# weigert/SoilMachine

Hardware: NVIDIA H100
Metric: particle-steps/sec (higher is better)
Workload: dtype f64

## Files before the change

soilmachine_b200/csrc/sm_device.cuh:

```cuda
#pragma once
#include <cuda_runtime.h>
#include "sm_core.cuh"

#ifdef SM_PROFILE
#define SM_PROF_DECL unsigned long long prof_[16] = {0}; long long pt_ = clock64();
#define SM_PROF(i) { long long t_ = clock64(); prof_[i] += (unsigned long long)(t_ - pt_); pt_ = t_; }
#define SM_PROF_FLUSH(ctl) { for (int i_ = 0; i_ < 16; i_++) if (prof_[i_]) atomicAdd(&(ctl)->prof[i_], prof_[i_]); }
#else
#define SM_PROF_DECL
#define SM_PROF(i)
#define SM_PROF_FLUSH(ctl)
#endif

struct PoolRing {
  unsigned long long head;
  unsigned long long tail;
};

struct RunCtl {
  unsigned int barrier;
  unsigned int alive_slot[3];
  unsigned int tag_base;
  unsigned int err;
  unsigned long long steps, sweeps, exit_oob, exit_evap, exit_stall, drops, alive;
// ... 96 lines not shown
__device__ __forceinline__ unsigned int ld_relaxed_sys_u32(const unsigned int* p) {
  unsigned int v;
  asm volatile("ld.relaxed.sys.global.u32 %0, [%1];" : "=r"(v) : "l"(p) : "memory");
  return v;
}
__device__ __forceinline__ unsigned long long ld_relaxed_sys_u64(const unsigned long long* p) {
  unsigned long long v;
  asm volatile("ld.relaxed.sys.global.u64 %0, [%1];" : "=l"(v) : "l"(p) : "memory");
  return v;
}
__device__ __forceinline__ void prefetch_l2(const void* p) { asm volatile("prefetch.global.L2 [%0];" ::"l"(p)); }
#ifndef SM_POLL_NS
#define SM_POLL_NS 0
#endif
__device__ __forceinline__ void poll_backoff() { if (SM_POLL_NS > 0) __nanosleep(SM_POLL_NS); }
__device__ __forceinline__ unsigned int ld_acquire_sys_u32(const unsigned int* p) {
  unsigned int v;
  asm volatile("ld.acquire.sys.global.u32 %0, [%1];" : "=r"(v) : "l"(p) : "memory");
  return v;
}
__device__ __forceinline__ void st_release_sys_u32(unsigned int* p, unsigned int v) {
  asm volatile("st.release.sys.global.u32 [%0], %1;" ::"l"(p), "r"(v) : "memory");
}

__device__ __forceinline__ unsigned long long ld_acquire_sys_u64(const unsigned long long* p) {
  unsigned long long v;
  asm volatile("ld.acquire.sys.global.u64 %0, [%1];" : "=l"(v) : "l"(p) : "memory");
  return v;
}
__device__ __forceinline__ void st_release_sys_u64(unsigned long long* p, unsigned long long v) {
  asm volatile("st.release.sys.global.u64 [%0], %1;" ::"l"(p), "l"(v) : "memory");
}

__device__ __forceinline__ void grid_barrier(unsigned int* counter, unsigned int& epoch) {
  __syncthreads();
  epoch++;
  if (threadIdx.x == 0) {
    __threadfence();
    atomicAdd(counter, 1u);
    const unsigned int target = epoch * gridDim.x;
    while ((int)(ld_relaxed_u32(counter) - target) < 0) poll_backoff();
    __threadfence();
  }
  __syncthreads();
}

__device__ __forceinline__ unsigned int grid_barrier_multi(const DevCtx& c, unsigned int& epoch, unsigned int gbase,
                                                           unsigned int local_alive_slot) {
  RunCtl* ctl = c.ctl;
  __syncthreads();
  epoch++;
  const unsigned int ge = gbase + epoch;
  if (threadIdx.x == 0) {
    __threadfence();
    atomicAdd(&ctl->barrier, 1u);
    if (blockIdx.x == 0) {
      const unsigned int target = epoch * gridDim.x;
      while ((int)(ld_acquire_u32(&ctl->barrier) - target) < 0) { }
      const unsigned int mine = ld_volatile_u32(&ctl->alive_slot[local_alive_slot]);
#ifdef SM_XBAR_FENCES
      for (int q = 0; q < c.nranks; q++) st_volatile_u32(&c.peer[q].ctl->xalive[ge & 1u][c.rank], mine);
      __threadfence_system();
      for (int q = 0; q < c.nranks; q++) st_volatile_u32(&c.peer[q].ctl->xflag[c.rank], ge);
      unsigned int total = 0;
      for (int q = 0; q < c.nranks; q++) {
        while ((int)(ld_volatile_u32(&ctl->xflag[q]) - ge) < 0) { }
      }
      __threadfence_system();
      for (int q = 0; q < c.nranks; q++) total += ld_volatile_u32(&ctl->xalive[ge & 1u][q]);
#else
      for (int q = 0; q < c.nranks; q++) st_volatile_u32(&c.peer[q].ctl->xalive[ge & 1u][c.rank], mine);
      for (int q = 0; q < c.nranks; q++) st_release_sys_u32(&c.peer[q].ctl->xflag[c.rank], ge);
      unsigned int total = 0;
      for (int q = 0; q < c.nranks; q++) {
        while ((int)(ld_acquire_sys_u32(&ctl->xflag[q]) - ge) < 0) { }
// ... 260 lines not shown
```

soilmachine_b200/csrc/sm_engine.cu:

```cuda
#include <cuda_runtime.h>
#include <stddef.h>
#include <stdio.h>
#include <stdlib.h>
#include <string.h>
#include <string>
#include <vector>
#include <algorithm>
#include "../../include/soilmachine_b200.h"
#include "../../include/soilmachine/soilfile.hpp"
#include "sm_device.cuh"
#include "sm_noise.cuh"
#include "sm_hydro.cuh"
#include "sm_lbm.cuh"

#define KIND_WATER 0
#define KIND_WIND 1

template <int KIND> struct Reach {
  static constexpr int D = (KIND == KIND_WATER) ? 6 : 10;
  static constexpr int G = (KIND == KIND_WATER) ? 8 : 16;
  static constexpr int STEP = (KIND == KIND_WATER) ? 2 : 3;
  static constexpr int RING = (KIND == KIND_WATER) ? 1 : 2;
};

// ... 1756 lines not shown
    if (mask & (1 << kind)) {
      for (int ls = lshift;; ls--) {
        const size_t sm2 = (size_t)(threads >> ls) * (SM_WIN_BYTES + SM_KX * 4);
        int occ = 0;
        if (kind == KIND_WATER) CK(cudaOccupancyMaxActiveBlocksPerMultiprocessor(&occ, k_run_exact<KIND_WATER>, threads, sm2));
        else CK(cudaOccupancyMaxActiveBlocksPerMultiprocessor(&occ, k_run_exact<KIND_WIND>, threads, sm2));
        const long long need_threads = (long long)std::max(n, 1) << ls;
        const long long maxblocks = (long long)ctx->num_sms * occ;
        if (occ >= 1 && (need_threads <= maxblocks * threads || ls == 0)) {
          use_exact = true; lshift = ls; smem = sm2;
          blocks = (int)std::max<long long>(1, std::min<long long>(maxblocks, (need_threads + threads - 1) / threads));
          break;
        }
        if (ls == 0) break;
      }
    }
  }
  bool use_coop = SM_DEFAULT_COOP || ctx->d.bud != nullptr || ctx->d.wind_v4 != nullptr;
  {
    const char* e = getenv("SM_KERNEL");
    if (e && strcmp(e, "thread") == 0) use_coop = false;
    if (e && strcmp(e, "warp") == 0) use_coop = true;
  }
  if (use_coop) {
    const int sw_warps = kind == KIND_WIND ? SwShape<KIND_WIND>::WARPS : SwShape<KIND_WATER>::WARPS;
    const int cthreads = sw_warps * 32;
    int occ = 0;
    const bool budget = ctx->d.bud != nullptr;
    bool exact = false;
    {
      const char* e = getenv("SM_EXACT");
      exact = (((e ? atoi(e) : SM_DEFAULT_EXACT) >> kind) & 1) != 0;
    }
    void* const fns[16] = {(void*)k_sweep<KIND_WATER, false, false, false>, (void*)k_sweep<KIND_WIND, false, false, false>,
                           (void*)k_sweep<KIND_WATER, true, false, false>,  (void*)k_sweep<KIND_WIND, true, false, false>,
                           (void*)k_sweep<KIND_WATER, false, true, false>,  (void*)k_sweep<KIND_WIND, false, true, false>,
                           (void*)k_sweep<KIND_WATER, true, true, false>,   (void*)k_sweep<KIND_WIND, true, true, false>,
                           (void*)k_sweep<KIND_WATER, false, false, true>,  (void*)k_sweep<KIND_WIND, false, false, true>,
                           (void*)k_sweep<KIND_WATER, true, false, true>,   (void*)k_sweep<KIND_WIND, true, false, true>,
                           (void*)k_sweep<KIND_WATER, false, true, true>,   (void*)k_sweep<KIND_WIND, false, true, true>,
                           (void*)k_sweep<KIND_WATER, true, true, true>,    (void*)k_sweep<KIND_WIND, true, true, true>};
    void* fn = fns[(exact ? 8 : 0) + (budget ? 4 : 0) + (multi ? 2 : 0) + (kind == KIND_WATER ? 0 : 1)];
    const size_t csmem = (size_t)2 * (((size_t)std::max(n, 1) + 31) / 32) * sizeof(unsigned int);
    if (csmem > 40 * 1024) CK(cudaFuncSetAttribute((const void*)fn, cudaFuncAttributeMaxDynamicSharedMemorySize, (int)csmem));
    CK(cudaOccupancyMaxActiveBlocksPerMultiprocessor(&occ, (const void*)fn, cthreads, csmem));
    if (occ < 1) return fail(ctx, SM_ERR_CUDA, "sweep kernel does not fit an SM");
    const long long maxblocks = std::max<long long>(1, (long long)ctx->num_sms * occ / ctx->share);
    const long long want = ((long long)std::max(n, 1) + sw_warps - 1) / sw_warps;
    const int cblocks = (int)std::max<long long>(1, std::min(maxblocks, want));
    DevCtx dd = ctx->d;
    int ms = max_sweeps;
    if (ms <= 0) ms = -1;
    if (max_sweeps == SM_SWEEPS_NONE) ms = 0;
    void* cargs[] = {&dd, &n, (void*)&d_spawn, &ms};
    CK(cudaMemsetAsync(ctx->d.ctl, 0, 4 * sizeof(unsigned int), ctx->stream));
    CK(cudaMemsetAsync(&ctx->d.ctl->ticket[0], 0, 3 * sizeof(unsigned int), ctx->stream));
    for (int i = 0; i < 3; i++)
      CK(cudaMemsetAsync(ctx->d.lmask[i], 0, ((size_t)ctx->max_particles / 32 + 2) * sizeof(unsigned int), ctx->stream));
    CK(cudaEventRecord(ctx->ev0, ctx->stream));
    CK(cudaLaunchCooperativeKernel(fn, dim3(cblocks), dim3(cthreads), cargs, csmem, ctx->stream));
    CK(cudaEventRecord(ctx->ev1, ctx->stream));
    ctx->launches++;
    ctx->timing_pending = true;
    return SM_OK;
  }
  DevCtx d = ctx->d;
  if (max_sweeps <= 0) max_sweeps = -1;
  if (max_sweeps == SM_SWEEPS_NONE) max_sweeps = 0;
  void* args[] = {&d, &n, (void*)&d_spawn, &max_sweeps, &lshift};
  CK(cudaMemsetAsync(ctx->d.ctl, 0, 4 * sizeof(unsigned int), ctx->stream));
  CK(cudaEventRecord(ctx->ev0, ctx->stream));
  if (multi && kind == KIND_WATER)
    CK(cudaLaunchCooperativeKernel((void*)k_run<KIND_WATER, true>, dim3(blocks), dim3(threads), args, smem, ctx->stream));
  else if (multi)
    CK(cudaLaunchCooperativeKernel((void*)k_run<KIND_WIND, true>, dim3(blocks), dim3(threads), args, smem, ctx->stream));
  else if (use_exact && kind == KIND_WATER)
    CK(cudaLaunchCooperativeKernel((void*)k_run_exact<KIND_WATER>, dim3(blocks), dim3(threads), args, smem, ctx->stream));
  else if (use_exact)
    CK(cudaLaunchCooperativeKernel((void*)k_run_exact<KIND_WIND>, dim3(blocks), dim3(threads), args, smem, ctx->stream));
  else if (kind == KIND_WATER)
    CK(cudaLaunchCooperativeKernel((void*)k_run<KIND_WATER, false>, dim3(blocks), dim3(threads), args, smem, ctx->stream));
// ... 547 lines not shown
```

soilmachine_b200/csrc/sm_sweep.cuh:

```cuda
#pragma once
#include "sm_coop.cuh"

template <int KIND> struct SwShape {
  static constexpr int WARPS = (KIND == KIND_WIND) ? 10 : 8;
  static constexpr int MINBLOCKS = (KIND == KIND_WIND) ? 2 : 3;
};
#define SM_SW_NEAR 31
#define SM_SW_NEARX 128

struct WarpDev {
  int lane;
  template <class F> __device__ __forceinline__ void each(int n, F f) {
    __syncwarp();
    if (lane < n) f(lane);
    __syncwarp();
  }
  template <class F> __device__ __forceinline__ unsigned int ballot(int n, F f) {
    __syncwarp();
    bool v = false;
    if (lane < n) v = f(lane);
    const unsigned int m = __ballot_sync(0xffffffffu, v);
    __syncwarp();
    return m;
  }
  template <class F> __device__ __forceinline__ void one(F f) {
    __syncwarp();
    if (lane == 0) f();
    __syncwarp();
  }
  __device__ __forceinline__ bool lead() const { return lane == 0; }
};

template <bool MULTI, bool BUDGET = false> struct DevBack {
  static constexpr bool kBudget = BUDGET;
  static constexpr bool kHydroHooks = false;
  __device__ __forceinline__ void air_mark(Sec32*, int, int) {}
  __device__ __forceinline__ void wet_mark(int, int) {}
  __device__ __forceinline__ double volume_factor() const { return c.volume_factor; }
  const DevCtx& c;
  const SoilDev* s_soils;
  unsigned int phase;
  int cur_q;
  __device__ __forceinline__ DevBack(const DevCtx& ctx, const SoilDev* ss, unsigned int tag)
      : c(ctx), s_soils(ss), phase(tag % 3u), cur_q(0) {}
  __device__ __forceinline__ int dimx() const { return c.dimx; }
  __device__ __forceinline__ int dimy() const { return c.dimy; }
  __device__ __forceinline__ int scale() const { return c.scale; }
  __device__ __forceinline__ const SoilDev* soilp(uint32_t t) const { return &s_soils[t]; }
  __device__ __forceinline__ Sec32* cell_ptr(int x, int y) const { return ::cell_ptr<MULTI>(c, x, y); }
  __device__ __forceinline__ void focus(int x, int) { if (MULTI) cur_q = owner_of_x<true>(c, x); }
  __device__ __forceinline__ Sec32 pool_load(uint32_t i) { return MULTI ? c.peer[cur_q].pool[i] : c.pool[i]; }
  __device__ __forceinline__ void pool_store(uint32_t i, const Sec32& r) {
    if (MULTI) c.peer[cur_q].pool[i] = r; else c.pool[i] = r;
  }
  __device__ uint32_t pool_alloc() {
    const unsigned int pr = (phase + 1u) % 3u;
    RunCtl* const ctl = MULTI ? c.peer[cur_q].ctl : c.ctl;
    uint32_t* const ring = MULTI ? c.peer[cur_q].ringbuf[pr] : c.ringbuf[pr];
    const unsigned long long cap = MULTI ? c.peer[cur_q].pool_cap : c.pool_cap;
    PoolRing* R = &ctl->ring[pr];
    const unsigned long long t = *((volatile unsigned long long*)&R->tail);
    if (*((volatile unsigned long long*)&R->head) < t) {
      const unsigned long long h = MULTI ? atomicAdd_system(&R->head, 1ull) : atomicAdd(&R->head, 1ull);
      if (h < t) return ring[h % cap];
// ... 15 lines not shown
  }
  __device__ __forceinline__ float wfreq(int i) const { return c.wfreq[i]; }
  __device__ __forceinline__ float wtrack(int i) const { return c.wtrack[i]; }
  __device__ __forceinline__ float windfreq(int i) const { return c.windfreq[i]; }
  __device__ __forceinline__ void set_wtrack(int i, float v) { c.wtrack[i] = v; }
  __device__ __forceinline__ void set_windfreq(int i, float v) { c.windfreq[i] = v; }
  __device__ __forceinline__ void note_transfer() {}
  __device__ __forceinline__ void pspeed(float px, float py, double height, float* ps) const {
    const WindField f{c.wind_v4, c.wind_nx, c.wind_ny, c.wind_nz, c.dimx, c.dimy, c.scale};
    wind_field_pspeed(f, px, py, height, ps);
  }
};

struct __align__(32) WarpSmem {
  CoopScratch cs;
  uint32_t blk[SM_SW_NEARX];
  uint32_t pred[12];
  uint32_t cnt;
  uint32_t m0[SM_SW_NEARX / 32];
  uint32_t n1[SM_SW_NEARX / 32];
  uint32_t remote;
  uint32_t succ;
  uint32_t blkxy[SM_SW_NEARX];
};

#ifndef SM_PREFETCH
#define SM_PREFETCH 1
#endif
__device__ __forceinline__ float next_dy(const WaterP& p) { return p.sy; }
__device__ __forceinline__ float next_dy(const WindP& p) { return p.sz; }
template <class W, class A> __device__ __forceinline__ int do_step_coop(W& w, A& a, WaterP& p) { return water_step_coop(w, a, p); }
template <class W, class A> __device__ __forceinline__ int do_step_coop(W& w, A& a, WindP& p) { return wind_step_coop(w, a, p); }

template <int KIND, bool MULTI, bool EXACT = false>
__device__ __forceinline__ uint32_t coop_scan(const DevCtx& c, WarpSmem& ws, int lane, unsigned int tag, int pid, int ix,
                                              int iy, int R) {
  const unsigned int par = tag & 1u;
  const int G = Reach<KIND>::G;
  const int nbx = (c.dimx + G - 1) / G, nby = (c.dimy + G - 1) / G;
  if (lane == 0) { ws.cnt = 0; ws.succ = 0; if (EXACT) ws.remote = 0; }
  if (EXACT && lane < SM_SW_NEARX / 32) ws.m0[lane] = 0;
  __syncwarp();
  if (lane < 9) {
    const int cx = ix / G + lane / 3 - 1, cy = iy / G + lane % 3 - 1;
    uint32_t best = SM_NIL;
    if (cx >= 0 && cx < nbx && cy >= 0 && cy < nby) {
      const int bq = MULTI ? owner_of_x<MULTI>(c, cx * G) : 0;
      const unsigned long long* hp = MULTI ? c.peer[bq].head[par] : c.head[par];
      const unsigned long long h = *((volatile const unsigned long long*)&hp[cx * nby + cy]);
      if ((unsigned int)(h >> 32) == tag) {
        const uint2* nodes = MULTI ? c.peer[bq].node[par] : c.node[par];
        const uint32_t qtag = MULTI ? ((uint32_t)bq << 28) : 0u;
        uint32_t j = (uint32_t)h;
        while (j != SM_NIL) {
          const uint2 nd = nodes[j];
          if (j > (uint32_t)pid) ws.succ = 1u;
          if (j < (uint32_t)pid) {
            if (best == SM_NIL || (j | qtag) > best) best = j | qtag;
            int dx = (int)(nd.y >> 18) - ix, dy = (int)((nd.y >> 4) & 0x3FFFu) - iy;
            const int D = R + (int)(nd.y & 0xFu);
            dx = dx < 0 ? -dx : dx;
            dy = dy < 0 ? -dy : dy;
            if (dx <= D && dy <= D) {
              const unsigned int at = atomicAdd(&ws.cnt, 1u);
              if (at < (EXACT ? SM_SW_NEARX : SM_SW_NEAR)) {
                ws.blk[at] = j | qtag;
                if (EXACT) {
                  ws.blkxy[at] = nd.y;
                  if (Foot<KIND>::box_hits_M((int)(nd.y >> 18) - ix, (int)((nd.y >> 4) & 0x3FFFu) - iy, (int)(nd.y & 0xFu)))
                    atomicOr(&ws.m0[at >> 5], 1u << (at & 31u));
                  if (MULTI && bq != c.rank) ws.remote = 1u;
                }
              }
            }
          }
          j = nd.x;
        }
      }
    }
    ws.pred[lane] = best;
  }
  __syncwarp();
  const unsigned int cnt = ws.cnt;
  if (cnt <= SM_SW_NEAR) {
    if (lane < (int)cnt) return ws.blk[lane];
    if (lane == 31) return ws.pred[4];
    return SM_NIL;
  }
  return lane < 9 ? ws.pred[lane] : SM_NIL;
}

template <bool MULTI>
__device__ __forceinline__ void coop_wait(const DevCtx& c, unsigned int tag, uint32_t tgt) {
  bool ok = (tgt == SM_NIL);
  const unsigned int* dp = nullptr;
  bool remote = false;
  if (!ok) {
    if (MULTI) {
      const int bq = (int)(tgt >> 28);
      dp = &c.peer[bq].done[tgt & 0x0FFFFFFFu];
      remote = (bq != c.rank);
    } else dp = &c.done[tgt];
  }
  const bool had = !ok;
  for (;;) {
    if (!ok) {
      const unsigned int v = remote ? ld_relaxed_sys_u32(dp) : ld_relaxed_u32(dp);
      ok = v >= tag;
    }
    if (__all_sync(0xffffffffu, ok)) break;
    poll_backoff();
  }
  if (had) { if (remote) (void)ld_acquire_sys_u32(dp); else (void)ld_acquire_u32(dp); }
}

#define SM_XSYNC_K 8
__device__ __forceinline__ unsigned int grid_barrier_x(const DevCtx& c, unsigned int& epoch, unsigned int gbase,
                                                       unsigned int local_alive_slot, bool global,
                                                       unsigned int* s_total) {
  RunCtl* ctl = c.ctl;
  __syncthreads();
  epoch++;
  const unsigned int ge = gbase + epoch;
  if (threadIdx.x < 32) {
    const int lane = threadIdx.x;
    unsigned int prev = 0;
    if (lane == 0) {
      __threadfence();
      prev = atomicAdd(&ctl->barrier, 1u);
      __threadfence();
    }
    prev = __shfl_sync(0xffffffffu, prev, 0);
    const int d = lane - c.rank;
    const bool involved = lane < c.nranks && (global || (d >= -1 && d <= 1));
    if (prev == epoch * gridDim.x - 1u) {
      const unsigned int mine = ld_volatile_u32(&ctl->alive_slot[local_alive_slot]);
      if (involved)
        st_release_sys_u64(&c.peer[lane].ctl->xw[ge & 1u][c.rank], ((unsigned long long)ge << 32) | mine);
    }
    unsigned int cnt = 0;
    bool ok = !involved;
    for (;;) {
      if (!ok) {
        const unsigned long long wv = ld_relaxed_sys_u64(&ctl->xw[ge & 1u][lane]);
        if ((int)((unsigned int)(wv >> 32) - ge) >= 0) { ok = true; cnt = (unsigned int)wv; }
      }
      if (__all_sync(0xffffffffu, ok)) break;
      poll_backoff();
    }
    if (involved) (void)ld_acquire_sys_u64(&ctl->xw[ge & 1u][lane]);
#pragma unroll
    for (int o = 16; o > 0; o >>= 1) cnt += __shfl_xor_sync(0xffffffffu, cnt, o);
    if (lane == 0) *s_total = cnt;
  }
  __syncthreads();
  return *s_total;
}

template <class W, class A> __device__ __forceinline__ int do_move_coop(W& w, A& a, WaterP& p, WaterMidCoop& m) { return water_move_coop(w, a, p, m, SM_CW_PLUS); }
template <class W, class A> __device__ __forceinline__ int do_move_coop(W& w, A& a, WindP& p, WindMidCoop& m) { return wind_move_coop(w, a, p, m, SM_CW_PLUS); }
template <class W, class A> __device__ __forceinline__ int do_interact_coop(W& w, A& a, WaterP& p, const WaterMidCoop& m) { return water_interact_coop(w, a, p, m); }
template <class W, class A> __device__ __forceinline__ int do_interact_coop(W& w, A& a, WindP& p, const WindMidCoop& m) { return wind_interact_coop(w, a, p, m); }
template <class W, class A> __device__ __forceinline__ int do_move_coop_full(W& w, A& a, WaterP& p, WaterMidCoop& m) { return water_move_coop(w, a, p, m, 0x1FFu); }
template <class W, class A> __device__ __forceinline__ int do_move_coop_full(W& w, A& a, WindP& p, WindMidCoop& m) { return wind_move_coop(w, a, p, m, 0x1FFu); }
template <int KIND> struct MidCoopType { typedef WaterMidCoop T; };
template <> struct MidCoopType<KIND_WIND> { typedef WindMidCoop T; };

template <int KIND, bool MULTI, bool BUDGET>
__device__ __forceinline__ int sweep_exact(const DevCtx& c, WarpSmem& ws, WarpDev& w, const SoilDev* s_soils,
                                           unsigned int tag, int pid, int ix, int iy, int myR,
                                           typename PType<KIND>::T& p, bool edge) {
  const int lane = w.lane;
  const unsigned int cnt = ws.cnt;
  const uint32_t ownpred = ws.pred[4];
  for (unsigned int base = 0; base < cnt; base += 32u) {
    const bool mine = base + (unsigned int)lane < cnt;
    const uint32_t j = mine ? (ws.blk[base + lane] & 0x0FFFFFFFu) : 0u;
    const uint32_t jxy = mine ? ws.blkxy[base + lane] : 0u;
    const int jx = (int)(jxy >> 18), jy = (int)((jxy >> 4) & 0x3FFFu);
    bool need1 = mine;
    bool need0 = mine && ((ws.m0[base >> 5] >> lane) & 1u);
    bool acq = false;
    for (;;) {
      if (need0) {
        if (ld_relaxed_u32(&c.fin[j]) >= tag) { need0 = false; need1 = false; acq = true; }
        else {
          const unsigned long long v = *((volatile unsigned long long*)&c.mv[j]);
          if ((unsigned int)(v >> 32) == tag) {
            const int mx = (int)((v >> 16) & 0xFFFFu), my = (int)(v & 0xFFFFu);
            if (!Foot<KIND>::W_hits_M(jx, jy, mx, my, ix, iy)) need0 = false;
          }
        }
      }
      if (!__any_sync(0xffffffffu, need0)) break;
      poll_backoff();
    }
    if (acq) (void)ld_acquire_u32(&c.fin[j]);
    const unsigned int left = __ballot_sync(0xffffffffu, need1);
    if (lane == 0) ws.n1[base >> 5] = left;
  }
  __syncwarp();
  DevBack<MULTI, BUDGET> back(c, s_soils, tag);
  CoopWin<DevBack<MULTI, BUDGET> > a(back, &ws.cs);
  typename MidCoopType<KIND>::T mid;
  int r = do_move_coop(w, a, p, mid);
  if (r == SM_ALIVE) {
    const int nx = (int)roundf(p.px), ny = (int)roundf(p.py);
    if (lane == 0)
      *((volatile unsigned long long*)&c.mv[pid]) = ((unsigned long long)tag << 32) | ((unsigned long long)nx << 16) | (unsigned long long)ny;
    for (unsigned int base = 0; base < cnt; base += 32u) {
      const unsigned int left = ws.n1[base >> 5];
      if (left == 0u) continue;
      bool need1 = (left >> lane) & 1u;
      const uint32_t j = need1 ? (ws.blk[base + lane] & 0x0FFFFFFFu) : 0u;
      const uint32_t jxy = need1 ? ws.blkxy[base + lane] : 0u;
      const int jx = (int)(jxy >> 18), jy = (int)((jxy >> 4) & 0x3FFFu), jR = (int)(jxy & 0xFu);
      int mx = 0, my = 0;
      bool moved = false;
      bool acq = false;
      for (;;) {
        if (need1) {
          if (ld_relaxed_u32(&c.fin[j]) >= tag) { need1 = false; acq = true; }
          else {
            if (!moved) {
              const unsigned long long v = *((volatile unsigned long long*)&c.mv[j]);
              if ((unsigned int)(v >> 32) == tag) { mx = (int)((v >> 16) & 0xFFFFu); my = (int)(v & 0xFFFFu); moved = true; }
            }
            const bool hit = moved ? Foot<KIND>::F_hits_F(ix, iy, nx, ny, jx, jy, mx, my)
                                   : Foot<KIND>::box_hits_F(ix, iy, nx, ny, jx, jy, jR);
            if (!hit) need1 = false;
          }
        }
        if (!__any_sync(0xffffffffu, need1)) break;
        poll_backoff();
      }
      if (acq) (void)ld_acquire_u32(&c.fin[j]);
    }
    r = do_interact_coop(w, a, p, mid);
    a.flush(w);
  }
  if (lane == 0) {
    const unsigned int pub = (r == SM_ALIVE) ? tag : 0xFFFFFFFFu;
    if (ws.succ) {
      const unsigned int* dp = nullptr;
      if (ownpred != SM_NIL) dp = MULTI ? &c.peer[ownpred >> 28].done[ownpred & 0x0FFFFFFFu] : &c.done[ownpred];
      if (!(MULTI && edge) && (dp == nullptr || ld_relaxed_u32(dp) >= tag)) {
        if (dp != nullptr) (void)ld_acquire_u32(dp);
        fence_acq_rel_gpu();
        st_relaxed_u32(&c.fin[pid], pub);
        st_relaxed_u32(&c.done[pid], pub);
      } else {
        st_release_u32(&c.fin[pid], pub);
        if (dp != nullptr) {
          while (ld_relaxed_u32(dp) < tag) poll_backoff();
          (void)ld_acquire_u32(dp);
        }
        if (MULTI && edge) st_release_sys_u32(&c.done[pid], pub);
        else st_release_u32(&c.done[pid], pub);
      }
    } else {
      st_volatile_u32(&c.fin[pid], pub);
      st_volatile_u32(&c.done[pid], pub);
    }
  }
  __syncwarp();
  return r;
}

template <int NWARPS>
__device__ __forceinline__ unsigned int live_total(const unsigned int* __restrict__ mask, int W, unsigned int* s_word,
                                                   unsigned int* s_pref, unsigned int* s_wsum) {
  const int T = NWARPS * 32;
  const int cw = (W + T - 1) / T;
  const int lo = threadIdx.x * cw, hi = (lo + cw < W) ? lo + cw : W;
  unsigned int local = 0;
  for (int i = lo; i < hi; i++) {
    const unsigned int wd = ld_relaxed_u32(&mask[i]);
    s_word[i] = wd;
    local += (unsigned int)__popc(wd);
  }
  unsigned int incl = local;
#pragma unroll
  for (int o = 1; o < 32; o <<= 1) {
    const unsigned int v = __shfl_up_sync(0xffffffffu, incl, o);
    if ((int)(threadIdx.x & 31) >= o) incl += v;
  }
  __syncthreads();
  if ((threadIdx.x & 31) == 31) s_wsum[threadIdx.x >> 5] = incl;
  __syncthreads();
  unsigned int base = 0, total = 0;
#pragma unroll
  for (int k = 0; k < NWARPS; k++) {
    const unsigned int v = s_wsum[k];
    if (k < (int)(threadIdx.x >> 5)) base += v;
    total += v;
  }
  unsigned int run = base + incl - local;
  for (int i = lo; i < hi; i++) { s_pref[i] = run; run += (unsigned int)__popc(s_word[i]); }
  __syncthreads();
  return total;
}

template <int KIND, bool MULTI, bool BUDGET, bool EXACT>
__global__ void __launch_bounds__(SwShape<KIND>::WARPS * 32, SwShape<KIND>::MINBLOCKS) k_sweep(DevCtx c, int n, const float* __restrict__ spawn,
                                                                            int max_sweeps) {
  typedef typename PType<KIND>::T P;
  constexpr int NWARPS = SwShape<KIND>::WARPS;
  __shared__ SoilDev s_soils[SM_MAX_SOILS];
  __shared__ unsigned int s_alive, s_total, s_wsum[NWARPS];
  __shared__ WarpSmem s_w[NWARPS];
  extern __shared__ unsigned int s_live[];
  const int W = (n + 31) >> 5;
  unsigned int* const s_word = s_live;
  unsigned int* const s_pref = s_live + W;
  for (int i = threadIdx.x; i < c.nsoils; i += blockDim.x) s_soils[i] = c.soils[i];
  if (threadIdx.x == 0) s_alive = 0;
  __syncthreads();

  RunCtl* ctl = c.ctl;
  unsigned int epoch = 0;
  const unsigned int tag0 = ctl->tag_base;
  const unsigned int gbase = MULTI ? ctl->epoch_base : 0u;
  const int gtid = blockIdx.x * blockDim.x + threadIdx.x;
  const int lane = threadIdx.x & 31;
  const int wib = threadIdx.x >> 5;
  const int slot = blockIdx.x * NWARPS + wib;
  const int nslots = gridDim.x * NWARPS;
  WarpSmem& ws = s_w[wib];
  WarpDev w{lane};

  unsigned long long n_steps = 0, n_oob = 0, n_evap = 0, n_stall = 0;
  bool any_doa = false;

  unsigned int total_alive = 0;
  {
    unsigned int my_alive = 0;
    unsigned long long doa = 0;
    const int nthreads = gridDim.x * blockDim.x;
    for (int pid = gtid; pid < n; pid += nthreads) {
      bool alive;
      if (spawn != nullptr) {
        const float x = spawn[2 * pid], y = spawn[2 * pid + 1];
        const int sx = (int)roundf(x), sy = (int)roundf(y);
        if (MULTI && owner_of_x<MULTI>(c, sx) != c.rank) {
          c.alive[pid] = 0;
          if (BUDGET) for (int k = 0; k < SM_BUDGET_SLOTS; k++) c.bud[(size_t)pid * SM_BUDGET_SLOTS + k] = 0.0;
          continue;
        }
        const uint32_t contains = s_soils[rec_surface(*cell_ptr<MULTI>(c, sx, sy))].transports;
        if (KIND == KIND_WATER) {
          WaterP q{x, y, 0.0f, 0.0f, 1.0, 0.0, contains};
          store_particle(c, pid, q);
          alive = true;
        } else {
          WindP q{x, y, -2.0f, 0.0f, 1.0f, 0.0, 0.0, contains};
          store_particle(c, pid, q);
          alive = !(s_soils[contains].suspension == 0.0);
          if (!alive) { doa++; any_doa = true; }
        }
        c.alive[pid] = alive ? 1 : 0;
        c.done[pid] = alive ? (tag0 - 1u) : 0xFFFFFFFFu;
        if (EXACT) c.fin[pid] = alive ? (tag0 - 1u) : 0xFFFFFFFFu;
        if (BUDGET) for (int k = 0; k < SM_BUDGET_SLOTS; k++) c.bud[(size_t)pid * SM_BUDGET_SLOTS + k] = 0.0;
      } else {
        alive = c.alive[pid] != 0;
      }
      if (alive) {
        P q;
        load_particle(c, pid, q);
        bin_insert<KIND, MULTI>(c, tag0, pid, (int)roundf(q.px), (int)roundf(q.py), particle_reach(q), c.rank);
        atomicOr(&c.lmask[tag0 % 3u][pid >> 5], 1u << (pid & 31));
        my_alive++;
      }
    }
    if (doa) atomicAdd(&ctl->exit_oob, doa);
    if (my_alive) atomicAdd(&s_alive, my_alive);
    __syncthreads();
    if (threadIdx.x == 0) {
      if (s_alive) atomicAdd(&ctl->alive_slot[0], s_alive);
      s_alive = 0;
    }
    if (MULTI) total_alive = grid_barrier_x(c, epoch, gbase, 0u, true, &s_total);
    else grid_barrier(&ctl->barrier, epoch);
  }
  const bool xnb = MULTI && c.strip_w >= 3 * Reach<KIND>::G;
  bool xglobal = true;
  int last_active = -1;

  int s = 0;
  for (;; s++) {
    const unsigned int tag = tag0 + (unsigned int)s;
    if (max_sweeps >= 0 && s >= max_sweeps) {
      if (!MULTI) total_alive = live_total<NWARPS>(c.lmask[tag % 3u], W, s_word, s_pref, s_wsum);
      break;
    }
    const unsigned int live = live_total<NWARPS>(c.lmask[tag % 3u], W, s_word, s_pref, s_wsum);
    if (!MULTI) total_alive = live;
    if ((!MULTI || xglobal) && total_alive == 0) break;
    {
      unsigned int* const z = c.lmask[(tag + 2u) % 3u];
      for (int i = gtid; i < W; i += gridDim.x * blockDim.x) z[i] = 0u;
    }
    if (gtid == 0) {
      if (MULTI) st_volatile_u32(&ctl->alive_slot[(s + 2) % 3], 0u);
      st_volatile_u32(&ctl->ticket[(tag + 2u) % 3u], 0u);
    }

    unsigned int my_alive = 0;
#ifdef SM_PROFILE
    unsigned long long prof_warp = 0;
    if (gtid == 0 && s < 16380) c.dbg[8 * s + 0] = live;
#endif
    {
    for (unsigned int rank = (unsigned int)slot; rank < live;) {
      int lo = 0, hi = W - 1;
      while (lo < hi) {
        const int mid = (lo + hi + 1) >> 1;
        if (s_pref[mid] <= rank) lo = mid; else hi = mid - 1;
      }
      const int pid = (lo << 5) + (int)__fns(s_word[lo], 0u, (int)(rank - s_pref[lo]) + 1);
      last_active = s;
#ifdef SM_PROFILE
      const long long pc0 = clock64();
      if (lane == 0 && s < 16380) {
        unsigned long long gt; asm volatile("mov.u64 %0, %%globaltimer;" : "=l"(gt));
        atomicMax(&c.dbg[8 * s + 6], ~gt);
      }
#endif
      P p;
      load_particle(c, pid, p);
      const int ix = (int)roundf(p.px), iy = (int)roundf(p.py);
      const int myR = particle_reach(p);
      const uint32_t tgt = coop_scan<KIND, MULTI, EXACT>(c, ws, lane, tag, pid, ix, iy, myR);
#ifdef SM_PROFILE
      const long long pc1 = clock64();
      long long pc2 = pc1;
#endif
      bool edge = false;
      if (MULTI) {
        const int xlo = c.rank * c.strip_w, xhi = xlo + c.strip_w;
        edge = (ix < xlo + 32 && c.rank > 0) || (ix >= xhi - 32 && c.rank < c.nranks - 1);
      }
      int r = SM_ALIVE;
      bool exact_now = false;
      if constexpr (EXACT) {
        exact_now = ws.cnt <= SM_SW_NEARX && !(MULTI && ws.remote);
        if (exact_now) r = sweep_exact<KIND, MULTI, BUDGET>(c, ws, w, s_soils, tag, pid, ix, iy, myR, p, edge);
      }
      if (!exact_now) {
        coop_wait<MULTI>(c, tag, tgt);
#ifdef SM_PROFILE
        pc2 = clock64();
#endif
        DevBack<MULTI, BUDGET> back(c, s_soils, tag);
        CoopWin<DevBack<MULTI, BUDGET> > a(back, &ws.cs);
#ifdef SM_PROFILE
        long long pcm, pci;
        {
          typename MidCoopType<KIND>::T mid;
          r = do_move_coop_full(w, a, p, mid);
          pcm = clock64();
          if (r == SM_ALIVE) r = do_interact_coop(w, a, p, mid);
          pci = clock64();
        }
#else
        r = do_step_coop(w, a, p);
#endif
        a.flush(w);
        if (lane == 0) {
          const unsigned int pub = (r == SM_ALIVE) ? tag : 0xFFFFFFFFu;
          if (ws.succ) {
            if (EXACT && !(MULTI && edge)) {
              fence_acq_rel_gpu();
              st_relaxed_u32(&c.fin[pid], pub);
              st_relaxed_u32(&c.done[pid], pub);
            } else {
              if (EXACT) st_release_u32(&c.fin[pid], pub);
              if (MULTI && edge) st_release_sys_u32(&c.done[pid], pub);
              else st_release_u32(&c.done[pid], pub);
            }
          } else {
            if (EXACT) st_volatile_u32(&c.fin[pid], pub);
            st_volatile_u32(&c.done[pid], pub);
// ... 21 lines not shown
          for (int k = 0; k < SM_BUDGET_SLOTS; k++) {
            const size_t at = (size_t)pid * SM_BUDGET_SLOTS + k;
            const double tot = c.bud[at] + ws.cs.acc[k];
            if (MULTI && bq != c.rank) c.bud[at] = 0.0;
            dst[at] = tot;
          }
        }
        if (r == SM_ALIVE) {
          int ddx = jx - ix, ddy = jy - iy;
          ddx = ddx < 0 ? -ddx : ddx; ddy = ddy < 0 ? -ddy : ddy;
          const int lim = myR - Reach<KIND>::RING;
          if (ddx > lim || ddy > lim) atomicOr(&ctl->err, 1u << 4);
          const int nq = owner_of_x<MULTI>(c, jx);
          if (MULTI && nq != c.rank) {
            DevCtx o = c;
            o.pa = c.peer[nq].pa; o.pb = c.peer[nq].pb; o.pc = c.peer[nq].pc;
            store_particle(o, pid, p);
            c.peer[nq].done[pid] = tag;
            if (EXACT) c.peer[nq].fin[pid] = tag;
            c.peer[nq].alive[pid] = 1;
            c.alive[pid] = 0;
            atomicOr_system(&c.peer[nq].lmask[(tag + 1u) % 3u][pid >> 5], 1u << (pid & 31));
          } else {
            store_particle(c, pid, p);
            atomicOr(&c.lmask[(tag + 1u) % 3u][pid >> 5], 1u << (pid & 31));
          }
          bin_insert<KIND, MULTI>(c, tag + 1u, pid, jx, jy, particle_reach(p), nq);
        } else {
          store_particle(c, pid, p);
          c.alive[pid] = 0;
        }
      }
#if SM_PREFETCH
      if (r == SM_ALIVE && lane < 18) {
        const int ox = lane < 9 ? jx : (int)roundf(p.px + p.sx);
        const int oy = lane < 9 ? jy : (int)roundf(p.py + next_dy(p));
        const int k = lane < 9 ? lane : lane - 9;
        const int x = ox + k / 3 - 1, y = oy + k % 3 - 1;
        if (x >= 0 && y >= 0 && x < c.dimx && y < c.dimy && (!MULTI || owner_of_x<MULTI>(c, x) == c.rank))
          prefetch_l2(cell_ptr<MULTI>(c, x, y));
      }
#endif
#ifdef SM_PROFILE
      {
        const long long pc3 = clock64();
        prof_warp += (unsigned long long)(pc3 - pc0);
        if (lane == 0 && s < 16380) {
          atomicMax(&c.dbg[8 * s + 1], (unsigned long long)(pc3 - pc2));
          atomicMax(&c.dbg[8 * s + 2], (unsigned long long)(pc2 - pc1));
          atomicAdd(&c.dbg[8 * s + 4], (unsigned long long)(pc3 - pc2));
          atomicAdd(&c.dbg[8 * s + 5], 1ull);
        }
      }
#endif
      if (r == SM_ALIVE) { n_steps++; my_alive++; }
      else if (r == SM_EXIT_OOB) n_oob++;
      else if (r == SM_EXIT_STALL) n_stall++;
      else { n_steps++; n_evap++; }
      __syncwarp();
      if (live <= (unsigned int)nslots) break;
      unsigned int nr = 0;
      if (lane == 0) nr = (unsigned int)nslots + atomicAdd(&ctl->ticket[tag % 3u], 1u);
      rank = __shfl_sync(0xffffffffu, nr, 0);
    }
    }
#ifdef SM_PROFILE
    if (lane == 0 && s < 16380 && prof_warp) {
      atomicMax(&c.dbg[8 * s + 3], prof_warp);
      unsigned long long gt; asm volatile("mov.u64 %0, %%globaltimer;" : "=l"(gt));
      atomicMax(&c.dbg[8 * s + 7], gt);
    }
#endif
    if (MULTI) {
      if (lane == 0 && my_alive) atomicAdd(&s_alive, my_alive);
      __syncthreads();
      if (threadIdx.x == 0) {
        if (s_alive) atomicAdd(&ctl->alive_slot[(s + 1) % 3], s_alive);
        s_alive = 0;
      }
    }
    if (MULTI) {
      xglobal = !xnb || ((s + 1) % SM_XSYNC_K == 0) || (max_sweeps >= 0 && s + 1 >= max_sweeps);
      total_alive = grid_barrier_x(c, epoch, gbase, (unsigned int)((s + 1) % 3), xglobal, &s_total);
    } else grid_barrier(&ctl->barrier, epoch);
  }

  if (lane == 0) {
    if (n_steps) atomicAdd(&ctl->steps, n_steps);
    if (n_oob) atomicAdd(&ctl->exit_oob, n_oob);
    if (n_evap) atomicAdd(&ctl->exit_evap, n_evap);
    if (n_stall) atomicAdd(&ctl->exit_stall, n_stall);
  }
  if (any_doa) atomicMax(&ctl->sweeps, 1ull);
  if (MULTI && lane == 0 && last_active >= 0) atomicMax(&ctl->sweeps, (unsigned long long)(last_active + 1));
  if (gtid == 0) {
    if (!MULTI) atomicMax(&ctl->sweeps, (unsigned long long)s);
    ctl->alive = total_alive;
    ctl->tag_base = tag0 + (unsigned int)s + 2u;
    if (MULTI) ctl->epoch_base = gbase + epoch;
  }
}
```

Measured before the change: 196.4 million.

## Add half-warp tile option for sweep kernel and lean barriers for wind

Makes the cooperative sweep kernel templated on tile width so each particle can be handled by 16 lanes instead of a full warp. Per-tile helpers loop over the extra indices and use masked ballots. The default tile stays at 32, so the tiling only takes effect when the SM_TILE environment variable is set. Separately, wind kernels now use a lean grid barrier (acquire load instead of a trailing threadfence) and skip one __syncthreads in live_total, which trims synchronization overhead in the default path for wind.

```diff
diff --git a/soilmachine_b200/csrc/sm_device.cuh b/soilmachine_b200/csrc/sm_device.cuh
--- a/soilmachine_b200/csrc/sm_device.cuh
+++ b/soilmachine_b200/csrc/sm_device.cuh
@@ -152,6 +152,7 @@
   asm volatile("st.release.sys.global.u64 [%0], %1;" ::"l"(p), "l"(v) : "memory");
 }
 
+template <bool LEAN = false>
 __device__ __forceinline__ void grid_barrier(unsigned int* counter, unsigned int& epoch) {
   __syncthreads();
   epoch++;
@@ -160,7 +161,8 @@
     atomicAdd(counter, 1u);
     const unsigned int target = epoch * gridDim.x;
     while ((int)(ld_relaxed_u32(counter) - target) < 0) poll_backoff();
-    __threadfence();
+    if (LEAN) (void)ld_acquire_u32(counter);
+    else __threadfence();
   }
   __syncthreads();
 }
diff --git a/soilmachine_b200/csrc/sm_engine.cu b/soilmachine_b200/csrc/sm_engine.cu
--- a/soilmachine_b200/csrc/sm_engine.cu
+++ b/soilmachine_b200/csrc/sm_engine.cu
@@ -1812,21 +1812,36 @@
       const char* e = getenv("SM_EXACT");
       exact = (((e ? atoi(e) : SM_DEFAULT_EXACT) >> kind) & 1) != 0;
     }
-    void* const fns[16] = {(void*)k_sweep<KIND_WATER, false, false, false>, (void*)k_sweep<KIND_WIND, false, false, false>,
-                           (void*)k_sweep<KIND_WATER, true, false, false>,  (void*)k_sweep<KIND_WIND, true, false, false>,
-                           (void*)k_sweep<KIND_WATER, false, true, false>,  (void*)k_sweep<KIND_WIND, false, true, false>,
-                           (void*)k_sweep<KIND_WATER, true, true, false>,   (void*)k_sweep<KIND_WIND, true, true, false>,
-                           (void*)k_sweep<KIND_WATER, false, false, true>,  (void*)k_sweep<KIND_WIND, false, false, true>,
-                           (void*)k_sweep<KIND_WATER, true, false, true>,   (void*)k_sweep<KIND_WIND, true, false, true>,
-                           (void*)k_sweep<KIND_WATER, false, true, true>,   (void*)k_sweep<KIND_WIND, false, true, true>,
-                           (void*)k_sweep<KIND_WATER, true, true, true>,    (void*)k_sweep<KIND_WIND, true, true, true>};
-    void* fn = fns[(exact ? 8 : 0) + (budget ? 4 : 0) + (multi ? 2 : 0) + (kind == KIND_WATER ? 0 : 1)];
+    bool tile16 = false;
+    {
+      const char* e = getenv("SM_TILE");
+      const int dflt = (SwShape<KIND_WATER>::TILE == 16 ? 1 : 0) | (SwShape<KIND_WIND>::TILE == 16 ? 2 : 0);
+      tile16 = (((e ? atoi(e) : dflt) >> kind) & 1) != 0;
+    }
+#define SM_SWEEP_FNS(T)                                                                                                 \
+  {(void*)k_sweep<KIND_WATER, false, false, false, T>, (void*)k_sweep<KIND_WIND, false, false, false, T>,             \
+   (void*)k_sweep<KIND_WATER, true, false, false, T>,  (void*)k_sweep<KIND_WIND, true, false, false, T>,              \
+   (void*)k_sweep<KIND_WATER, false, true, false, T>,  (void*)k_sweep<KIND_WIND, false, true, false, T>,              \
+   (void*)k_sweep<KIND_WATER, true, true, false, T>,   (void*)k_sweep<KIND_WIND, true, true, false, T>,               \
+   (void*)k_sweep<KIND_WATER, false, false, true, T>,  (void*)k_sweep<KIND_WIND, false, false, true, T>,              \
+   (void*)k_sweep<KIND_WATER, true, false, true, T>,   (void*)k_sweep<KIND_WIND, true, false, true, T>,               \
+   (void*)k_sweep<KIND_WATER, false, true, true, T>,   (void*)k_sweep<KIND_WIND, false, true, true, T>,               \
+   (void*)k_sweep<KIND_WATER, true, true, true, T>,    (void*)k_sweep<KIND_WIND, true, true, true, T>}
+    void* const fns[2][16] = {SM_SWEEP_FNS(32), SM_SWEEP_FNS(16)};
+#undef SM_SWEEP_FNS
+    void* fn = fns[tile16 ? 1 : 0][(exact ? 8 : 0) + (budget ? 4 : 0) + (multi ? 2 : 0) + (kind == KIND_WATER ? 0 : 1)];
+    const int sw_tiles = sw_warps * (tile16 ? 2 : 1);
     const size_t csmem = (size_t)2 * (((size_t)std::max(n, 1) + 31) / 32) * sizeof(unsigned int);
-    if (csmem > 40 * 1024) CK(cudaFuncSetAttribute((const void*)fn, cudaFuncAttributeMaxDynamicSharedMemorySize, (int)csmem));
+    {
+      cudaFuncAttributes fa;
+      CK(cudaFuncGetAttributes(&fa, (const void*)fn));
+      if (fa.sharedSizeBytes + csmem > 48 * 1024)
+        CK(cudaFuncSetAttribute((const void*)fn, cudaFuncAttributeMaxDynamicSharedMemorySize, (int)csmem));
+    }
     CK(cudaOccupancyMaxActiveBlocksPerMultiprocessor(&occ, (const void*)fn, cthreads, csmem));
     if (occ < 1) return fail(ctx, SM_ERR_CUDA, "sweep kernel does not fit an SM");
     const long long maxblocks = std::max<long long>(1, (long long)ctx->num_sms * occ / ctx->share);
-    const long long want = ((long long)std::max(n, 1) + sw_warps - 1) / sw_warps;
+    const long long want = ((long long)std::max(n, 1) + sw_tiles - 1) / sw_tiles;
     const int cblocks = (int)std::max<long long>(1, std::min(maxblocks, want));
     DevCtx dd = ctx->d;
     int ms = max_sweeps;
diff --git a/soilmachine_b200/csrc/sm_sweep.cuh b/soilmachine_b200/csrc/sm_sweep.cuh
--- a/soilmachine_b200/csrc/sm_sweep.cuh
+++ b/soilmachine_b200/csrc/sm_sweep.cuh
@@ -4,32 +4,64 @@
 template <int KIND> struct SwShape {
   static constexpr int WARPS = (KIND == KIND_WIND) ? 10 : 8;
   static constexpr int MINBLOCKS = (KIND == KIND_WIND) ? 2 : 3;
+  static constexpr int TILE = 32;
 };
 #define SM_SW_NEAR 31
 #define SM_SW_NEARX 128
 
-struct WarpDev {
+template <int T> struct TileDev {
+  static_assert(T == 16 || T == 32, "tile width");
+  static constexpr int R = 32 / T;
   int lane;
+  unsigned int mask;
+  __device__ __forceinline__ explicit TileDev(int l)
+      : lane(l), mask(T == 32 ? 0xffffffffu : (((1u << T) - 1u) << (threadIdx.x & 31u & ~(unsigned int)(T - 1)))) {}
   template <class F> __device__ __forceinline__ void each(int n, F f) {
-    __syncwarp();
-    if (lane < n) f(lane);
-    __syncwarp();
+    __syncwarp(mask);
+    if constexpr (T == 32) {
+      if (lane < n) f(lane);
+    } else {
+#pragma unroll
+      for (int r = 0; r < R; r++)
+        if (r * T + lane < n) f(r * T + lane);
+    }
+    __syncwarp(mask);
   }
   template <class F> __device__ __forceinline__ unsigned int ballot(int n, F f) {
-    __syncwarp();
-    bool v = false;
-    if (lane < n) v = f(lane);
-    const unsigned int m = __ballot_sync(0xffffffffu, v);
-    __syncwarp();
+    __syncwarp(mask);
+    unsigned int m;
+    if constexpr (T == 32) {
+      bool v = false;
+      if (lane < n) v = f(lane);
+      m = __ballot_sync(0xffffffffu, v);
+    } else {
+      bool v[R];
+#pragma unroll
+      for (int r = 0; r < R; r++) {
+        v[r] = false;
+        if (r * T + lane < n) v[r] = f(r * T + lane);
+      }
+      const unsigned int sh = threadIdx.x & 31u & ~(unsigned int)(T - 1);
+      m = 0;
+#pragma unroll
+      for (int r = 0; r < R; r++)
+        if (r * T < n) m |= ((__ballot_sync(mask, v[r]) >> sh) & ((1u << T) - 1u)) << (r * T);
+    }
+    __syncwarp(mask);
     return m;
   }
   template <class F> __device__ __forceinline__ void one(F f) {
-    __syncwarp();
+    __syncwarp(mask);
     if (lane == 0) f();
-    __syncwarp();
+    __syncwarp(mask);
   }
   __device__ __forceinline__ bool lead() const { return lane == 0; }
+  __device__ __forceinline__ unsigned int vote(bool v) const {
+    if constexpr (T == 32) return __ballot_sync(0xffffffffu, v);
+    else return (__ballot_sync(mask, v) >> (threadIdx.x & 31u & ~(unsigned int)(T - 1))) & ((1u << T) - 1u);
+  }
 };
+typedef TileDev<32> WarpDev;
 
 template <bool MULTI, bool BUDGET = false> struct DevBack {
   static constexpr bool kBudget = BUDGET;
@@ -111,15 +143,26 @@
 template <class W, class A> __device__ __forceinline__ int do_step_coop(W& w, A& a, WaterP& p) { return water_step_coop(w, a, p); }
 template <class W, class A> __device__ __forceinline__ int do_step_coop(W& w, A& a, WindP& p) { return wind_step_coop(w, a, p); }
 
-template <int KIND, bool MULTI, bool EXACT = false>
-__device__ __forceinline__ uint32_t coop_scan(const DevCtx& c, WarpSmem& ws, int lane, unsigned int tag, int pid, int ix,
-                                              int iy, int R) {
+__device__ __forceinline__ uint32_t scan_target(const WarpSmem& ws, unsigned int cnt, int i) {
+  if (cnt <= SM_SW_NEAR) {
+    if (i < (int)cnt) return ws.blk[i];
+    if (i == 31) return ws.pred[4];
+    return SM_NIL;
+  }
+  return i < 9 ? ws.pred[i] : SM_NIL;
+}
+template <int T> struct WaitSet { uint32_t t[32 / T]; };
+
+template <int KIND, bool MULTI, bool EXACT, int T>
+__device__ __forceinline__ auto coop_scan(const DevCtx& c, WarpSmem& ws, const TileDev<T>& w, unsigned int tag,
+                                                int pid, int ix, int iy, int R) {
+  const int lane = w.lane;
   const unsigned int par = tag & 1u;
   const int G = Reach<KIND>::G;
   const int nbx = (c.dimx + G - 1) / G, nby = (c.dimy + G - 1) / G;
   if (lane == 0) { ws.cnt = 0; ws.succ = 0; if (EXACT) ws.remote = 0; }
   if (EXACT && lane < SM_SW_NEARX / 32) ws.m0[lane] = 0;
-  __syncwarp();
+  __syncwarp(w.mask);
   if (lane < 9) {
     const int cx = ix / G + lane / 3 - 1, cy = iy / G + lane % 3 - 1;
     uint32_t best = SM_NIL;
@@ -159,18 +202,25 @@
     }
     ws.pred[lane] = best;
   }
-  __syncwarp();
+  __syncwarp(w.mask);
   const unsigned int cnt = ws.cnt;
-  if (cnt <= SM_SW_NEAR) {
-    if (lane < (int)cnt) return ws.blk[lane];
-    if (lane == 31) return ws.pred[4];
-    return SM_NIL;
-  }
-  return lane < 9 ? ws.pred[lane] : SM_NIL;
+  if constexpr (T == 32) {
+    if (cnt <= SM_SW_NEAR) {
+      if (lane < (int)cnt) return ws.blk[lane];
+      if (lane == 31) return ws.pred[4];
+      return (uint32_t)SM_NIL;
+    }
+    return lane < 9 ? ws.pred[lane] : (uint32_t)SM_NIL;
+  } else {
+    WaitSet<T> ts;
+#pragma unroll
+    for (int r = 0; r < 32 / T; r++) ts.t[r] = scan_target(ws, cnt, r * T + lane);
+    return ts;
+  }
 }
 
 template <bool MULTI>
-__device__ __forceinline__ void coop_wait(const DevCtx& c, unsigned int tag, uint32_t tgt) {
+__device__ __forceinline__ void coop_wait(const DevCtx& c, unsigned int tag, uint32_t tgt, unsigned int) {
   bool ok = (tgt == SM_NIL);
   const unsigned int* dp = nullptr;
   bool remote = false;
@@ -191,6 +241,36 @@
     poll_backoff();
   }
   if (had) { if (remote) (void)ld_acquire_sys_u32(dp); else (void)ld_acquire_u32(dp); }
+}
+template <bool MULTI, int T>
+__device__ __forceinline__ void coop_wait(const DevCtx& c, unsigned int tag, const WaitSet<T>& ts, unsigned int mask) {
+  constexpr int R = 32 / T;
+  auto word = [&](uint32_t t) -> const unsigned int* {
+    return MULTI ? &c.peer[t >> 28].done[t & 0x0FFFFFFFu] : &c.done[t];
+  };
+  auto remote = [&](uint32_t t) { return MULTI && (int)(t >> 28) != c.rank; };
+  bool ok[R];
+#pragma unroll
+  for (int r = 0; r < R; r++) ok[r] = (ts.t[r] == SM_NIL);
+  for (;;) {
+    bool all = true;
+#pragma unroll
+    for (int r = 0; r < R; r++) {
+      if (!ok[r]) {
+        const uint32_t t = ts.t[r];
+        const unsigned int v = remote(t) ? ld_relaxed_sys_u32(word(t)) : ld_relaxed_u32(word(t));
+        ok[r] = v >= tag;
+      }
+      all = all && ok[r];
+    }
+    if (__all_sync(mask, all)) break;
+    poll_backoff();
+  }
+#pragma unroll
+  for (int r = 0; r < R; r++) {
+    const uint32_t t = ts.t[r];
+    if (t != SM_NIL) { if (remote(t)) (void)ld_acquire_sys_u32(word(t)); else (void)ld_acquire_u32(word(t)); }
+  }
 }
 
 #define SM_XSYNC_K 8
@@ -245,20 +325,21 @@
 template <int KIND> struct MidCoopType { typedef WaterMidCoop T; };
 template <> struct MidCoopType<KIND_WIND> { typedef WindMidCoop T; };
 
-template <int KIND, bool MULTI, bool BUDGET>
-__device__ __forceinline__ int sweep_exact(const DevCtx& c, WarpSmem& ws, WarpDev& w, const SoilDev* s_soils,
+template <int KIND, bool MULTI, bool BUDGET, int T>
+__device__ __forceinline__ int sweep_exact(const DevCtx& c, WarpSmem& ws, TileDev<T>& w, const SoilDev* s_soils,
                                            unsigned int tag, int pid, int ix, int iy, int myR,
                                            typename PType<KIND>::T& p, bool edge) {
   const int lane = w.lane;
   const unsigned int cnt = ws.cnt;
   const uint32_t ownpred = ws.pred[4];
-  for (unsigned int base = 0; base < cnt; base += 32u) {
+  for (unsigned int base = 0; base < cnt; base += (unsigned int)T) {
+    const unsigned int sh = (T == 32) ? 0u : (base & 31u);
     const bool mine = base + (unsigned int)lane < cnt;
     const uint32_t j = mine ? (ws.blk[base + lane] & 0x0FFFFFFFu) : 0u;
     const uint32_t jxy = mine ? ws.blkxy[base + lane] : 0u;
     const int jx = (int)(jxy >> 18), jy = (int)((jxy >> 4) & 0x3FFFu);
     bool need1 = mine;
-    bool need0 = mine && ((ws.m0[base >> 5] >> lane) & 1u);
+    bool need0 = mine && ((ws.m0[base >> 5] >> (sh + lane)) & 1u);
     bool acq = false;
     for (;;) {
       if (need0) {
@@ -271,14 +352,17 @@
           }
         }
       }
-      if (!__any_sync(0xffffffffu, need0)) break;
+      if (!__any_sync(w.mask, need0)) break;
       poll_backoff();
     }
     if (acq) (void)ld_acquire_u32(&c.fin[j]);
-    const unsigned int left = __ballot_sync(0xffffffffu, need1);
-    if (lane == 0) ws.n1[base >> 5] = left;
-  }
-  __syncwarp();
+    const unsigned int left = w.vote(need1);
+    if (lane == 0) {
+      if (sh == 0u) ws.n1[base >> 5] = left;
+      else ws.n1[base >> 5] |= left << sh;
+    }
+  }
+  __syncwarp(w.mask);
   DevBack<MULTI, BUDGET> back(c, s_soils, tag);
   CoopWin<DevBack<MULTI, BUDGET> > a(back, &ws.cs);
   typename MidCoopType<KIND>::T mid;
@@ -287,8 +371,8 @@
     const int nx = (int)roundf(p.px), ny = (int)roundf(p.py);
     if (lane == 0)
       *((volatile unsigned long long*)&c.mv[pid]) = ((unsigned long long)tag << 32) | ((unsigned long long)nx << 16) | (unsigned long long)ny;
-    for (unsigned int base = 0; base < cnt; base += 32u) {
-      const unsigned int left = ws.n1[base >> 5];
+    for (unsigned int base = 0; base < cnt; base += (unsigned int)T) {
+      const unsigned int left = (T == 32) ? ws.n1[base >> 5] : ((ws.n1[base >> 5] >> (base & 31u)) & ((1u << (T & 31)) - 1u));
       if (left == 0u) continue;
       bool need1 = (left >> lane) & 1u;
       const uint32_t j = need1 ? (ws.blk[base + lane] & 0x0FFFFFFFu) : 0u;
@@ -310,7 +394,7 @@
             if (!hit) need1 = false;
           }
         }
-        if (!__any_sync(0xffffffffu, need1)) break;
+        if (!__any_sync(w.mask, need1)) break;
         poll_backoff();
       }
       if (acq) (void)ld_acquire_u32(&c.fin[j]);
@@ -342,11 +426,11 @@
       st_volatile_u32(&c.done[pid], pub);
     }
   }
-  __syncwarp();
+  __syncwarp(w.mask);
   return r;
 }
 
-template <int NWARPS>
+template <int NWARPS, bool LEAN = false>
 __device__ __forceinline__ unsigned int live_total(const unsigned int* __restrict__ mask, int W, unsigned int* s_word,
                                                    unsigned int* s_pref, unsigned int* s_wsum) {
   const int T = NWARPS * 32;
@@ -364,7 +448,7 @@
     const unsigned int v = __shfl_up_sync(0xffffffffu, incl, o);
     if ((int)(threadIdx.x & 31) >= o) incl += v;
   }
-  __syncthreads();
+  if (!LEAN) __syncthreads();
   if ((threadIdx.x & 31) == 31) s_wsum[threadIdx.x >> 5] = incl;
   __syncthreads();
   unsigned int base = 0, total = 0;
@@ -380,14 +464,15 @@
   return total;
 }
 
-template <int KIND, bool MULTI, bool BUDGET, bool EXACT>
+template <int KIND, bool MULTI, bool BUDGET, bool EXACT, int TILE>
 __global__ void __launch_bounds__(SwShape<KIND>::WARPS * 32, SwShape<KIND>::MINBLOCKS) k_sweep(DevCtx c, int n, const float* __restrict__ spawn,
                                                                             int max_sweeps) {
   typedef typename PType<KIND>::T P;
   constexpr int NWARPS = SwShape<KIND>::WARPS;
+  constexpr int NTILES = NWARPS * 32 / TILE;
   __shared__ SoilDev s_soils[SM_MAX_SOILS];
   __shared__ unsigned int s_alive, s_total, s_wsum[NWARPS];
-  __shared__ WarpSmem s_w[NWARPS];
+  __shared__ WarpSmem s_w[NTILES];
   extern __shared__ unsigned int s_live[];
   const int W = (n + 31) >> 5;
   unsigned int* const s_word = s_live;
@@ -401,12 +486,12 @@
   const unsigned int tag0 = ctl->tag_base;
   const unsigned int gbase = MULTI ? ctl->epoch_base : 0u;
   const int gtid = blockIdx.x * blockDim.x + threadIdx.x;
-  const int lane = threadIdx.x & 31;
-  const int wib = threadIdx.x >> 5;
-  const int slot = blockIdx.x * NWARPS + wib;
-  const int nslots = gridDim.x * NWARPS;
-  WarpSmem& ws = s_w[wib];
-  WarpDev w{lane};
+  const int lane = threadIdx.x & (TILE - 1);
+  const int tib = threadIdx.x / TILE;
+  const int slot = blockIdx.x * NTILES + tib;
+  const int nslots = gridDim.x * NTILES;
+  WarpSmem& ws = s_w[tib];
+  TileDev<TILE> w(lane);
 
   unsigned long long n_steps = 0, n_oob = 0, n_evap = 0, n_stall = 0;
   bool any_doa = false;
@@ -460,7 +545,7 @@
       s_alive = 0;
     }
     if (MULTI) total_alive = grid_barrier_x(c, epoch, gbase, 0u, true, &s_total);
-    else grid_barrier(&ctl->barrier, epoch);
+    else grid_barrier<KIND == KIND_WIND>(&ctl->barrier, epoch);
   }
   const bool xnb = MULTI && c.strip_w >= 3 * Reach<KIND>::G;
   bool xglobal = true;
@@ -470,10 +555,10 @@
   for (;; s++) {
     const unsigned int tag = tag0 + (unsigned int)s;
     if (max_sweeps >= 0 && s >= max_sweeps) {
-      if (!MULTI) total_alive = live_total<NWARPS>(c.lmask[tag % 3u], W, s_word, s_pref, s_wsum);
+      if (!MULTI) total_alive = live_total<NWARPS, KIND == KIND_WIND>(c.lmask[tag % 3u], W, s_word, s_pref, s_wsum);
       break;
     }
-    const unsigned int live = live_total<NWARPS>(c.lmask[tag % 3u], W, s_word, s_pref, s_wsum);
+    const unsigned int live = live_total<NWARPS, KIND == KIND_WIND>(c.lmask[tag % 3u], W, s_word, s_pref, s_wsum);
     if (!MULTI) total_alive = live;
     if ((!MULTI || xglobal) && total_alive == 0) break;
     {
@@ -510,7 +595,7 @@
       load_particle(c, pid, p);
       const int ix = (int)roundf(p.px), iy = (int)roundf(p.py);
       const int myR = particle_reach(p);
-      const uint32_t tgt = coop_scan<KIND, MULTI, EXACT>(c, ws, lane, tag, pid, ix, iy, myR);
+      const auto tgt = coop_scan<KIND, MULTI, EXACT>(c, ws, w, tag, pid, ix, iy, myR);
 #ifdef SM_PROFILE
       const long long pc1 = clock64();
       long long pc2 = pc1;
@@ -527,7 +612,7 @@
         if (exact_now) r = sweep_exact<KIND, MULTI, BUDGET>(c, ws, w, s_soils, tag, pid, ix, iy, myR, p, edge);
       }
       if (!exact_now) {
-        coop_wait<MULTI>(c, tag, tgt);
+        coop_wait<MULTI>(c, tag, tgt, w.mask);
 #ifdef SM_PROFILE
         pc2 = clock64();
 #endif
@@ -615,13 +700,17 @@
         }
       }
 #if SM_PREFETCH
-      if (r == SM_ALIVE && lane < 18) {
-        const int ox = lane < 9 ? jx : (int)roundf(p.px + p.sx);
-        const int oy = lane < 9 ? jy : (int)roundf(p.py + next_dy(p));
-        const int k = lane < 9 ? lane : lane - 9;
-        const int x = ox + k / 3 - 1, y = oy + k % 3 - 1;
-        if (x >= 0 && y >= 0 && x < c.dimx && y < c.dimy && (!MULTI || owner_of_x<MULTI>(c, x) == c.rank))
-          prefetch_l2(cell_ptr<MULTI>(c, x, y));
+#pragma unroll
+      for (int rd = 0; rd < (18 + TILE - 1) / TILE; rd++) {
+        const int l = rd * TILE + lane;
+        if (r == SM_ALIVE && l < 18) {
+          const int ox = l < 9 ? jx : (int)roundf(p.px + p.sx);
+          const int oy = l < 9 ? jy : (int)roundf(p.py + next_dy(p));
+          const int k = l < 9 ? l : l - 9;
+          const int x = ox + k / 3 - 1, y = oy + k % 3 - 1;
+          if (x >= 0 && y >= 0 && x < c.dimx && y < c.dimy && (!MULTI || owner_of_x<MULTI>(c, x) == c.rank))
+            prefetch_l2(cell_ptr<MULTI>(c, x, y));
+        }
       }
 #endif
 #ifdef SM_PROFILE
@@ -640,11 +729,12 @@
       else if (r == SM_EXIT_OOB) n_oob++;
       else if (r == SM_EXIT_STALL) n_stall++;
       else { n_steps++; n_evap++; }
-      __syncwarp();
+      __syncwarp(w.mask);
       if (live <= (unsigned int)nslots) break;
       unsigned int nr = 0;
       if (lane == 0) nr = (unsigned int)nslots + atomicAdd(&ctl->ticket[tag % 3u], 1u);
-      rank = __shfl_sync(0xffffffffu, nr, 0);
+      if constexpr (TILE == 32) rank = __shfl_sync(0xffffffffu, nr, 0);
+      else rank = __shfl_sync(w.mask, nr, 0, TILE);
     }
     }
 #ifdef SM_PROFILE
@@ -665,7 +755,7 @@
     if (MULTI) {
       xglobal = !xnb || ((s + 1) % SM_XSYNC_K == 0) || (max_sweeps >= 0 && s + 1 >= max_sweeps);
       total_alive = grid_barrier_x(c, epoch, gbase, (unsigned int)((s + 1) % 3), xglobal, &s_total);
-    } else grid_barrier(&ctl->barrier, epoch);
+    } else grid_barrier<KIND == KIND_WIND>(&ctl->barrier, epoch);
   }
 
   if (lane == 0) {
```

Result: faster. 198.6 million (median of 6 runs) (+1.1%).
